# hhlgt/erasure-codes-prototype

Hardware: AMD Instinct MI355X
Metric: GiB/s encode + single-block decode (device-resident), RS(10,4) 1 MiB blocks, 1 & 8 GPU (higher is better)
Workload: dtype u8; 1 GPU; RS(10,4) encode + rotating 1-erasure decode (e = s mod 14); block_size=1048576, stripes_per_gpu=4096, global_stripes=4096, parallelism=stripes sharded over 1 GPU(s), no data-path collective

## Files before the change

erasure-codes-prototype_amd/csrc/gf_device.hpp:

```cpp
#pragma once
#include "gf_kernels.hpp"

namespace ecg {

#define ECG_CONST __attribute__((address_space(4)))
template <typename T>
__device__ __forceinline__ const ECG_CONST T* cst(const T* p) {
    return (const ECG_CONST T*)p;
}

template <int MODE>
__device__ __forceinline__ const uint8_t* src_ptr(const GfLaunch& a, int s, int prog, int j) {
    if constexpr (MODE == GF_MODE_INLINE || MODE == GF_MODE_INLINE_LAT) {
        return a.isrc[j];
    } else if constexpr (MODE == GF_MODE_PTRS) {
        return cst(a.src_ptrs)[(size_t)s * a.k + j];
    } else {
        const long long sa = a.stripe_of ? (long long)cst(a.stripe_of)[s] : (long long)s;
        return a.in_base + sa * a.in_sstride + (long long)cst(a.src_ids)[prog * a.k + j] * a.in_bstride;
    }
}

__device__ __forceinline__ uint32_t perm(uint32_t hi, uint32_t lo, uint32_t sel) {
    return __builtin_amdgcn_perm(hi, lo, sel);
}

__device__ __forceinline__ uint32_t xor3(uint32_t a, uint32_t b, uint32_t c) {
    return __builtin_amdgcn_bitop3_b32(a, b, c, 0x96);
}

typedef uint32_t u32x4 __attribute__((ext_vector_type(4)));

template <int NT>
__device__ __forceinline__ void load16(const uint8_t* p, uint32_t (&x)[4]) {
    u32x4 v;
    if constexpr (NT & 1) v = __builtin_nontemporal_load(reinterpret_cast<const u32x4*>(p));
    else v = *reinterpret_cast<const u32x4*>(p);
    x[0] = v.x; x[1] = v.y; x[2] = v.z; x[3] = v.w;
}

struct Split {
    uint32_t i0, i1, i2;
};

__device__ __forceinline__ Split split(uint32_t x) {
    return {x & 0x07070707u, (x >> 3) & 0x07070707u, (x >> 6) & 0x03030303u};
}

__device__ __forceinline__ uint32_t gmul(const ECG_CONST CoefTab& t, const Split& s) {
    return xor3(perm(t.t0hi, t.t0lo, s.i0), perm(t.t1hi, t.t1lo, s.i1), perm(t.t2, t.t2, s.i2));
}

template <int MT, int U>
__device__ __forceinline__ void fold_general(const uint32_t (&x)[U][4], const ECG_CONST CoefTab* t,
                                             uint32_t (&acc)[MT][4]) {
#pragma unroll
    for (int u = 0; u + 1 < U; u += 2) {
#pragma unroll
        for (int d = 0; d < 4; ++d) {
            const Split s0 = split(x[u][d]);
            const Split s1 = split(x[u + 1][d]);
#pragma unroll
            for (int p = 0; p < MT; ++p)
                acc[p][d] = xor3(acc[p][d], gmul(t[u * MT + p], s0), gmul(t[(u + 1) * MT + p], s1));
        }
    }
    if constexpr (U & 1) {
#pragma unroll
        for (int d = 0; d < 4; ++d) {
            const Split s0 = split(x[U - 1][d]);
#pragma unroll
            for (int p = 0; p < MT; ++p) acc[p][d] ^= gmul(t[(U - 1) * MT + p], s0);
        }
    }
}

template <int MT, int U>
__device__ __forceinline__ void fold_binary(const uint32_t (&x)[U][4], const ECG_CONST CoefTab* t,
                                            uint32_t (&acc)[MT][4]) {
#pragma unroll
    for (int u = 0; u < U; ++u)
#pragma unroll
        for (int p = 0; p < MT; ++p) {
            const uint32_t msk = t[u * MT + p].mask;
#pragma unroll
            for (int d = 0; d < 4; ++d) acc[p][d] = __builtin_amdgcn_bitop3_b32(acc[p][d], x[u][d], msk, 0x78);
        }
}

template <int MT, int U, bool BIN>
__device__ __forceinline__ void fold(const uint32_t (&x)[U][4], const ECG_CONST CoefTab* t, uint32_t (&acc)[MT][4]) {
    if constexpr (BIN) fold_binary<MT, U>(x, t, acc);
    else fold_general<MT, U>(x, t, acc);
}

constexpr int occupancy_for(int MT) {
#ifdef ECG_OCC_OVERRIDE
    return MT <= 4 ? ECG_OCC_OVERRIDE : 4;
#else
    return MT <= 2 ? 8 : MT <= 4 ? 6 : MT == 5 ? 3 : 4;
#endif
}

__device__ __forceinline__ void wg_coords(const GfLaunch& a, int& s, int& w) {
    long long b = blockIdx.x;
    if (a.grid_map == 1) {
        const long long G = (long long)gridDim.x;
        const long long per = G >> 3;
        b = (b & 7) * per + (b >> 3);
    } else if (a.grid_map == 2) {
        const long long i = b >> 3;
        const long long ls = i / a.wg_per_stripe;
        const long long G = a.map_group;
        s = (int)(((ls / G) * 8 + (b & 7)) * G + ls % G);
        w = (int)(i - ls * a.wg_per_stripe);
        return;
    }
    s = (int)(b / a.wg_per_stripe);
    w = (int)(b - (long long)s * a.wg_per_stripe);
}

template <int MODE>
__device__ __forceinline__ int launch_prog(const GfLaunch& a, int& s) {
    int r = 0;
    if constexpr (MODE == GF_MODE_STRIDED) {
        if (a.row_split) {
            r = s % a.row_split;
            s = s / a.row_split;
        }
    }
    const int p = a.prog_of_stripe ? cst(a.prog_of_stripe)[s] : 0;
    if constexpr (MODE == GF_MODE_STRIDED) return a.row_split ? p * a.row_split + r : p;
    return p;
}

#ifdef ECG_TUNE_LOAD_BATCH
constexpr int kLoadBatch = ECG_TUNE_LOAD_BATCH;
#else
constexpr int kLoadBatch = 4;
#endif
#ifdef ECG_TUNE_GEN_WIDE_LB
constexpr int kGenWideLB = ECG_TUNE_GEN_WIDE_LB;
#else
constexpr int kGenWideLB = 2;
#endif
#ifdef ECG_TUNE_GEN_LB
constexpr int kGenLB = ECG_TUNE_GEN_LB;
#else
constexpr int kGenLB = 4;
#endif

}
```

erasure-codes-prototype_amd/csrc/gf_kernels.hip:

```cpp
#include <atomic>

#include "gf_kernels.hpp"
#include "gf256.hpp"

#if defined(__HIP_DEVICE_COMPILE__) && !defined(__gfx950__)
#error "gf_kernels.hip is gfx950 (CDNA4) code"
#endif

#include "gf_done_flag.hpp"
#include "gf_device.hpp"

namespace ecg {

namespace {

template <int MODE>
__device__ __forceinline__ uint8_t* dst_ptr(const GfLaunch& a, int s, int prog, int p) {
    if constexpr (MODE == GF_MODE_INLINE || MODE == GF_MODE_INLINE_LAT) {
        return a.idst[p];
    } else if constexpr (MODE == GF_MODE_PTRS) {
        return cst(a.dst_ptrs)[(size_t)s * a.m + p];
    } else {
        const long long sa = a.stripe_of ? (long long)cst(a.stripe_of)[s] : (long long)s;
        return a.out_base + sa * a.out_sstride + (long long)cst(a.dst_ids)[prog * a.m + p] * a.out_bstride;
    }
}

template <int NT>
__device__ __forceinline__ void store16(uint8_t* p, const uint32_t (&x)[4]) {
    u32x4 v;
    v.x = x[0]; v.y = x[1]; v.z = x[2]; v.w = x[3];
    if constexpr (NT & 2) __builtin_nontemporal_store(v, reinterpret_cast<u32x4*>(p));
    else *reinterpret_cast<u32x4*>(p) = v;
}

template <int MT, int MODE, int NT, bool BIN>
__global__ void __launch_bounds__(kThreads, MODE == GF_MODE_INLINE_LAT ? 1 : occupancy_for(MT)) gf_vec_kernel(const GfLaunch a) {
    int s, w;
    wg_coords(a, s, w);
    const int rt = blockIdx.y;
    const int prog = launch_prog<MODE>(a, s);
    const int k = a.k;
    const int row0 = rt * MT;
    const int nrows = min(MT, a.m - row0);
    const ECG_CONST CoefTab* T = cst(a.tabs) + (size_t)(prog * a.rtiles + rt) * (size_t)k * MT;
    const long long ncols = a.B >> 4;
    const long long c0 = (long long)w * a.cols_per_wg;
    const long long c1 = min(c0 + (long long)a.cols_per_wg, ncols);

    uint8_t* dst[MT];
#pragma unroll
    for (int p = 0; p < MT; ++p) dst[p] = (p < nrows) ? dst_ptr<MODE>(a, s, prog, row0 + p) : nullptr;

    for (long long c = c0 + threadIdx.x; c < c1; c += kThreads) {
        const long long off = c << 4;
        uint32_t acc[MT][4];
#pragma unroll
        for (int p = 0; p < MT; ++p)
#pragma unroll
            for (int d = 0; d < 4; ++d) acc[p][d] = 0u;

        int j = 0;
        if constexpr (MODE == GF_MODE_INLINE_LAT) {
            if (k <= 8) {
                uint32_t x[8][4];
#pragma unroll
                for (int u = 0; u < 8; ++u) load16<NT>(src_ptr<MODE>(a, s, prog, u < k ? u : 0) + off, x[u]);
#pragma unroll
                for (int u = 0; u < 8; ++u)
                    if (u < k) fold<MT, 1, BIN>(reinterpret_cast<const uint32_t(&)[1][4]>(x[u]), T + (size_t)u * MT, acc);
                j = k;
            } else if (k <= 16) {
                uint32_t x[16][4];
#pragma unroll
                for (int u = 0; u < 16; ++u) load16<NT>(src_ptr<MODE>(a, s, prog, u < k ? u : 0) + off, x[u]);
#pragma unroll
                for (int u = 0; u < 16; ++u)
                    if (u < k) fold<MT, 1, BIN>(reinterpret_cast<const uint32_t(&)[1][4]>(x[u]), T + (size_t)u * MT, acc);
                j = k;
            }
        }
        constexpr int LB = BIN ? kLoadBatch : MT >= 5 ? kGenWideLB : kGenLB;
        for (; j + LB <= k; j += LB) {
            uint32_t x[LB][4];
#pragma unroll
            for (int u = 0; u < LB; ++u) load16<NT>(src_ptr<MODE>(a, s, prog, j + u) + off, x[u]);
            fold<MT, LB, BIN>(x, T + (size_t)j * MT, acc);
        }
        if constexpr (LB > 4) {
            if (j + 4 <= k) {
                uint32_t x[4][4];
#pragma unroll
                for (int u = 0; u < 4; ++u) load16<NT>(src_ptr<MODE>(a, s, prog, j + u) + off, x[u]);
                fold<MT, 4, BIN>(x, T + (size_t)j * MT, acc);
                j += 4;
            }
        }
        if (j + 2 <= k) {
            uint32_t x[2][4];
#pragma unroll
            for (int u = 0; u < 2; ++u) load16<NT>(src_ptr<MODE>(a, s, prog, j + u) + off, x[u]);
            fold<MT, 2, BIN>(x, T + (size_t)j * MT, acc);
            j += 2;
        }
        if (j < k) {
            uint32_t x[1][4];
            load16<NT>(src_ptr<MODE>(a, s, prog, j) + off, x[0]);
            fold<MT, 1, BIN>(x, T + (size_t)j * MT, acc);
        }
#pragma unroll
        for (int p = 0; p < MT; ++p)
            if (p < nrows) store16<NT>(dst[p] + off, acc[p]);
    }
    if constexpr (MODE == GF_MODE_INLINE_LAT) {
        if (a.done_flags) post_done_flag(a);
    }
}

template <int MT, int KB>
struct LatTabs {
    static constexpr int kPieces = KB * MT * 2;
    static constexpr int kPerLane = (kPieces + 63) / 64;
    CoefTab t[kLatThreads / 64][KB * MT];
};

template <int KB, int MT>
struct LatArgs {
    const CoefTab* tabs;
    unsigned* done_flags;
    long long B;
    int k, m;
    unsigned done_seq;
    const uint8_t* src[KB];
    uint8_t* dst[MT];
};

template <int MT, int KB>
__device__ __forceinline__ void lat_tabs_load(const LatArgs<KB, MT>& a, u32x4 (&tv)[LatTabs<MT, KB>::kPerLane]) {
    const u32x4* src = reinterpret_cast<const u32x4*>(a.tabs);
    const int last = a.k * MT * 2 - 1;
    const int lane = threadIdx.x & 63;
#pragma unroll
    for (int i = 0; i < LatTabs<MT, KB>::kPerLane; ++i) tv[i] = src[min(lane + 64 * i, last)];
}

template <int MT, int KB>
__device__ __forceinline__ const CoefTab* lat_tabs_store(LatTabs<MT, KB>& lds,
                                                         const u32x4 (&tv)[LatTabs<MT, KB>::kPerLane]) {
    const int wave = threadIdx.x >> 6, lane = threadIdx.x & 63;
    u32x4* dst = reinterpret_cast<u32x4*>(lds.t[wave]);
#pragma unroll
    for (int i = 0; i < LatTabs<MT, KB>::kPerLane; ++i)
        if (lane + 64 * i < LatTabs<MT, KB>::kPieces) dst[lane + 64 * i] = tv[i];
    return lds.t[wave];
}

template <int MT, bool BIN, int KB>
__device__ __forceinline__ void lat_fold_lds(const int k, const CoefTab* T, const uint32_t (&x)[KB],
                                             uint32_t (&acc)[MT]) {
    struct R {
        uint32_t t0lo, t0hi, t1lo, t1hi, t2;
    };
    auto rd = [&](int u, R (&r)[MT]) {
        const CoefTab* t = T + (size_t)(u < k ? u : 0) * MT;
#pragma unroll
        for (int p = 0; p < MT; ++p) {
            if constexpr (BIN) r[p].t0lo = t[p].mask;
            else r[p] = {t[p].t0lo, t[p].t0hi, t[p].t1lo, t[p].t1hi, t[p].t2};
        }
    };
#pragma unroll
    for (int p = 0; p < MT; ++p) acc[p] = 0u;
    R cur[MT], nxt[MT];
    rd(0, cur);
#pragma unroll
    for (int u = 0; u < KB; ++u) {
        if (u + 1 < KB) rd(u + 1, nxt);
        const uint32_t keep = u < k ? ~0u : 0u;
        if constexpr (BIN) {
#pragma unroll
            for (int p = 0; p < MT; ++p) acc[p] = __builtin_amdgcn_bitop3_b32(acc[p], x[u], cur[p].t0lo & keep, 0x78);
        } else {
            const Split sp = split(x[u]);
#pragma unroll
            for (int p = 0; p < MT; ++p) {
                const uint32_t g = xor3(perm(cur[p].t0hi, cur[p].t0lo, sp.i0), perm(cur[p].t1hi, cur[p].t1lo, sp.i1),
                                        perm(cur[p].t2, cur[p].t2, sp.i2));
                acc[p] = __builtin_amdgcn_bitop3_b32(acc[p], g, keep, 0x78);
            }
        }
#pragma unroll
        for (int p = 0; p < MT; ++p) asm volatile("" : "+v"(acc[p]) : : "memory");
        if (u + 1 < KB)
#pragma unroll
            for (int p = 0; p < MT; ++p) cur[p] = nxt[p];
    }
}

__device__ __forceinline__ void lat_store(uint32_t* p, uint32_t v) {
#ifdef ECG_TUNE_LAT_STORE_SC1
    asm volatile("global_store_dword %0, %1, off sc0 sc1" ::"v"(p), "v"(v) : "memory");
#else
    __builtin_nontemporal_store(v, p);
#endif
}

template <int MT, bool BIN, int KB, bool EAGER>
__global__ void __launch_bounds__(kLatThreads, 1) gf_lat_dword_kernel(const LatArgs<KB, MT> a) {
    __shared__ LatTabs<MT, KB> lds;
    const int k = a.k;
    const int nrows = a.m;
    const long long ndw = a.B >> 2;
    const long long c = (long long)blockIdx.x * kLatThreads + threadIdx.x;
    const uint8_t* src[KB];
#pragma unroll
    for (int u = 0; u < KB; ++u) src[u] = a.src[u];
    uint8_t* dst[MT];
#pragma unroll
    for (int p = 0; p < MT; ++p) dst[p] = a.dst[p];
    unsigned* const flags = a.done_flags;
    u32x4 tv[LatTabs<MT, KB>::kPerLane];
    lat_tabs_load<MT, KB>(a, tv);
    __builtin_amdgcn_sched_barrier(0);
    const bool live = c < ndw;
    const long long off = (live ? c : ndw - 1) << 2;
    uint32_t x[KB];
#pragma unroll
    for (int u = 0; u < KB; ++u) x[u] = __builtin_nontemporal_load(reinterpret_cast<const uint32_t*>(src[u] + off));
    if constexpr (EAGER) __builtin_amdgcn_sched_barrier(0);
    const CoefTab* T = lat_tabs_store<MT, KB>(lds, tv);
    uint32_t acc[MT];
    lat_fold_lds<MT, BIN, KB>(k, T, x, acc);
    if (live) {
#pragma unroll
        for (int p = 0; p < MT; ++p)
            if (p < nrows) lat_store(reinterpret_cast<uint32_t*>(dst[p] + off), acc[p]);
    }
    if (flags) post_done_flag(flags + blockIdx.x, a.done_seq);
}


__device__ __forceinline__ unsigned long long wk_ptr(const unsigned* d, int q) {
    return ((unsigned long long)d[worker_pos(q + 1)] << 32) | d[worker_pos(q)];
}

template <int MT, bool BIN, int KB>
__device__ __forceinline__ void worker_call(const unsigned* d, CoefTab* wt) {
    const int k = (int)d[worker_pos(WF_K)];
    const int m = (int)d[worker_pos(WF_M)];
    const long long ndw = (long long)d[worker_pos(WF_B)] >> 2;
    const u32x4* tg = reinterpret_cast<const u32x4*>((uintptr_t)wk_ptr(d, WF_TABS));
    const uint8_t* in[KB];
#pragma unroll
    for (int u = 0; u < KB; u++) in[u] = (const uint8_t*)(uintptr_t)wk_ptr(d, WF_IN + 2 * (u < k ? u : 0));
    uint8_t* out[MT];
#pragma unroll
    for (int p = 0; p < MT; p++) out[p] = (uint8_t*)(uintptr_t)wk_ptr(d, WF_OUT + 2 * (p < m ? p : 0));
    constexpr int kPieces = KB * MT * 2, kPerLane = (kPieces + 63) / 64;
    const int last = k * MT * 2 - 1, lane = threadIdx.x & 63;
    u32x4 tv[kPerLane];
#pragma unroll
    for (int i = 0; i < kPerLane; ++i) tv[i] = tg[min(lane + 64 * i, last)];
    __builtin_amdgcn_sched_barrier(0);
    const long long stride = (long long)gridDim.x * kLatThreads;
    long long c = (long long)blockIdx.x * kLatThreads + threadIdx.x;
    const bool live = c < ndw;
    uint32_t x[KB];
#pragma unroll
    for (int u = 0; u < KB; u++) x[u] = __builtin_nontemporal_load(reinterpret_cast<const uint32_t*>(in[u]) + (live ? c : 0));
#pragma unroll
    for (int i = 0; i < kPerLane; ++i)
        if (lane + 64 * i < kPieces) reinterpret_cast<u32x4*>(wt)[lane + 64 * i] = tv[i];
    uint32_t acc[MT];
    lat_fold_lds<MT, BIN, KB>(k, wt, x, acc);
    if (live) {
#pragma unroll
        for (int p = 0; p < MT; p++)
            if (p < m) __builtin_nontemporal_store(acc[p], reinterpret_cast<uint32_t*>(out[p]) + c);
    }
    for (c += stride; c < ndw; c += stride) {
#pragma unroll
        for (int u = 0; u < KB; u++) x[u] = __builtin_nontemporal_load(reinterpret_cast<const uint32_t*>(in[u]) + c);
        lat_fold_lds<MT, BIN, KB>(k, wt, x, acc);
#pragma unroll
        for (int p = 0; p < MT; p++)
            if (p < m) __builtin_nontemporal_store(acc[p], reinterpret_cast<uint32_t*>(out[p]) + c);
    }
}

template <int MT, bool BIN>
__device__ __forceinline__ void worker_call_k(const unsigned* d, CoefTab* wt) {
    const unsigned k = d[worker_pos(WF_K)];
    if (k <= 4) worker_call<MT, BIN, 4>(d, wt);
    else if (k <= 6) worker_call<MT, BIN, 6>(d, wt);
    else if (k <= 8) worker_call<MT, BIN, 8>(d, wt);
    else if (k <= 10) worker_call<MT, BIN, 10>(d, wt);
    else if (k <= 12) worker_call<MT, BIN, 12>(d, wt);
    else worker_call<MT, BIN, 16>(d, wt);
}

template <bool BIN>
__device__ __forceinline__ void worker_call_m(const unsigned* d, CoefTab* wt) {
    switch (d[worker_pos(WF_M)]) {
        case 1: worker_call_k<1, BIN>(d, wt); break;
        case 2: worker_call_k<2, BIN>(d, wt); break;
        case 3: worker_call_k<3, BIN>(d, wt); break;
        default: worker_call_k<4, BIN>(d, wt); break;
    }
}

__global__ void __launch_bounds__(kLatThreads, 1) gf_call_worker_kernel(const WorkerArgs a) {
    __shared__ unsigned d[64];
    __shared__ unsigned go;
    __shared__ CoefTab wtabs[kLatThreads / 64][kWorkerMaxSrc * kWorkerMaxRows];
    const int tid = threadIdx.x;
    const bool leader = blockIdx.x == 0;
    unsigned next = a.start_seq;
    const unsigned long long t0 = wall_clock64();
    unsigned long long last = t0;
    const unsigned long long my_idle = leader ? a.idle_ticks : 2 * a.idle_ticks;
    const unsigned long long my_life = leader ? a.life_ticks : 2 * a.life_ticks;
    for (unsigned polls = 0; polls < a.max_polls; polls++) {
        const unsigned slot = next % (unsigned)kWorkerSlots;
        if (leader) {
            if (tid < 64) {
                const unsigned v = __hip_atomic_load(&a.ring[slot].w[tid], __ATOMIC_RELAXED, __HIP_MEMORY_SCOPE_SYSTEM);
                const unsigned stop = __hip_atomic_load(a.stop, __ATOMIC_RELAXED, __HIP_MEMORY_SCOPE_SYSTEM);
                d[tid] = v;
                if (tid == 0) go = stop ? 2u : 0u;
            }
            __syncthreads();
            if (tid == 0 && go == 0) {
                const unsigned long long t = wall_clock64();
                if (t - t0 > my_life) go = 2;
                else if (d[0] == next && d[16] == next && d[32] == next && d[48] == next) go = 1;
                else if (t - last > my_idle) go = 2;
            }
            __syncthreads();
            if (go == 1 && gridDim.x > 1 && tid < 64) {
                __hip_atomic_store(&a.mbox[slot].w[tid], d[tid], __ATOMIC_RELAXED, __HIP_MEMORY_SCOPE_AGENT);
                if (tid == 0) __hip_atomic_store(&a.mbseq[slot], next, __ATOMIC_RELEASE, __HIP_MEMORY_SCOPE_AGENT);
            }
        } else {
            if (tid == 0) {
                const unsigned sq = __hip_atomic_load(&a.mbseq[slot], __ATOMIC_ACQUIRE, __HIP_MEMORY_SCOPE_AGENT);
                const unsigned ex = __hip_atomic_load(&a.mbseq[kWorkerSlots], __ATOMIC_RELAXED, __HIP_MEMORY_SCOPE_AGENT);
                const unsigned long long t = wall_clock64();
                go = sq == next ? 1u : (ex == a.gen || t - last > my_idle || t - t0 > my_life) ? 2u : 0u;
            }
            __syncthreads();
            if (go == 1 && tid < 64)
                d[tid] = __hip_atomic_load(&a.mbox[slot].w[tid], __ATOMIC_RELAXED, __HIP_MEMORY_SCOPE_AGENT);
            __syncthreads();
        }
        const unsigned g = go;
        if (g == 2) break;
        if (g == 0) {
            __syncthreads();
            continue;
        }
        __builtin_amdgcn_fence(__ATOMIC_ACQUIRE, "");
        CoefTab* const wt = wtabs[tid >> 6];
        if (d[worker_pos(WF_BINARY)]) worker_call_m<true>(d, wt);
        else worker_call_m<false>(d, wt);
        post_done_flag(a.flags + (size_t)slot * kWorkerMaxWG + blockIdx.x, next);
        next++;
        last = wall_clock64();
        __syncthreads();
    }
    if (tid == 0) {
        if (leader) __hip_atomic_store(&a.mbseq[kWorkerSlots], a.gen, __ATOMIC_RELAXED, __HIP_MEMORY_SCOPE_AGENT);
        __hip_atomic_store(a.exit_info + blockIdx.x, a.gen, __ATOMIC_RELAXED, __HIP_MEMORY_SCOPE_SYSTEM);
    }
}

template <int MT, int MODE, bool BIN>
__global__ void __launch_bounds__(kThreads) gf_byte_kernel(const GfLaunch a) {
    int s, w;
    wg_coords(a, s, w);
    const int rt = blockIdx.y;
    const int prog = launch_prog<MODE>(a, s);
    const int k = a.k;
    const int row0 = rt * MT;
    const int nrows = min(MT, a.m - row0);
    const ECG_CONST CoefTab* T = cst(a.tabs) + (size_t)(prog * a.rtiles + rt) * (size_t)k * MT;
    const long long b0 = a.off0 + (long long)w * a.cols_per_wg;
    const long long b1 = min(b0 + (long long)a.cols_per_wg, a.B);
    for (long long o = b0 + threadIdx.x; o < b1; o += kThreads) {
        uint32_t acc[MT];
#pragma unroll
        for (int p = 0; p < MT; ++p) acc[p] = 0u;
        for (int j = 0; j < k; ++j) {
            const uint32_t x = src_ptr<MODE>(a, s, prog, j)[o];
            const ECG_CONST CoefTab* t = T + (size_t)j * MT;
            if constexpr (BIN) {
#pragma unroll
                for (int p = 0; p < MT; ++p) acc[p] ^= x & t[p].mask;
            } else {
                const Split sp = split(x);
#pragma unroll
                for (int p = 0; p < MT; ++p) acc[p] ^= gmul(t[p], sp);
            }
        }
#pragma unroll
        for (int p = 0; p < MT; ++p)
            if (p < nrows) dst_ptr<MODE>(a, s, prog, row0 + p)[o] = (uint8_t)(acc[p] & 0xffu);
    }
}

__global__ void __launch_bounds__(kThreads) fill_splitmix_kernel(uint8_t* dst, long long nbytes,
                                                                 unsigned long long seed,
                                                                 unsigned long long word_offset) {
    const long long nwords = nbytes >> 3;
    const long long stride = (long long)gridDim.x * kThreads;
    for (long long w = (long long)blockIdx.x * kThreads + threadIdx.x; w < ((nbytes + 7) >> 3); w += stride) {
        unsigned long long z = seed + (word_offset + (unsigned long long)w) * 0x9E3779B97F4A7C15ull;
        z = (z ^ (z >> 30)) * 0xBF58476D1CE4E5B9ull;
        z = (z ^ (z >> 27)) * 0x94D049BB133111EBull;
        z ^= z >> 31;
        if (w < nwords) {
            reinterpret_cast<unsigned long long*>(dst)[w] = z;
        } else {
            for (long long b = w * 8; b < nbytes; ++b) dst[b] = (uint8_t)(z >> (8 * (b - w * 8)));
        }
    }
}


std::atomic<long long> g_opt[ECG_OPT_COUNT] = {};
std::atomic<int> g_opt_init{0};

void init_options() {
    if (g_opt_init.load(std::memory_order_acquire)) return;
    auto env = [](const char* n, long long d) {
        const char* e = getenv(n);
        return e ? atoll(e) : d;
    };
    g_opt[ECG_OPT_NT].store(env("ECG_NT", 3));
    g_opt[ECG_OPT_COLS_PER_WG].store(env("ECG_COLS_PER_WG", 0));
    g_opt[ECG_OPT_GRID_MAP].store(env("ECG_GRID_MAP", 3));
    g_opt[ECG_OPT_ZEROCOPY_BYTES].store(env("ECG_ZEROCOPY_BYTES", 8 << 20));
    g_opt[ECG_OPT_PROGRAM_CACHE].store(env("ECG_PROGRAM_CACHE", 4096));
    g_opt[ECG_OPT_MAP_GROUP].store(env("ECG_MAP_GROUP", 1));
    g_opt[ECG_OPT_LAT_DWORD_BYTES].store(env("ECG_LAT_DWORD_BYTES", 1 << 20));
    g_opt[ECG_OPT_CALL_WORKER].store(env("ECG_CALL_WORKER", 0));
    g_opt[ECG_OPT_ROW_SPLIT].store(env("ECG_ROW_SPLIT", 16));
    g_opt[ECG_OPT_GRAVEYARD].store(env("ECG_GRAVEYARD", 16384));
    g_opt[ECG_OPT_MT1_LDS_PAD].store(env("ECG_MT1_LDS_PAD", -1));
    g_opt_init.store(1, std::memory_order_release);
}

using Launcher = hipError_t (*)(const GfLaunch&, dim3, hipStream_t);

template <typename T>
struct NoDeduce {
    using type = T;
};

template <typename... P>
hipError_t launch_kernel_lds(void (*kernel)(P...), dim3 grid, dim3 block, unsigned lds, hipStream_t st,
                             typename NoDeduce<P>::type... args) {
    void* argv[] = {(void*)&args...};
    return hipLaunchKernel((const void*)kernel, grid, block, argv, lds, st);
}

template <typename... P>
hipError_t launch_kernel(void (*kernel)(P...), dim3 grid, dim3 block, hipStream_t st,
                         typename NoDeduce<P>::type... args) {
    return launch_kernel_lds(kernel, grid, block, 0, st, args...);
}

template <typename F>
hipError_t launch_with(F kernel, const GfLaunch& a, dim3 grid, hipStream_t st) {
    return launch_kernel(kernel, grid, dim3(kThreads), st, a);
}

unsigned mt1_lds_pad(int k, bool ptrs) {
    const long long opt = g_opt[ECG_OPT_MT1_LDS_PAD].load(std::memory_order_relaxed);
    if (opt >= 0) return (unsigned)opt;
    if (k <= 1) return 0;
    if (k <= 3) return 12288;
    if (k == 4) return 16384;
    if (k == 5) return 0;
    if (k == 6) return ptrs ? 22528 : 20480;
    if (k == 7 || k == 9 || k == 10) return 22528;
    return 24576;
}

unsigned mt2_lds_pad(int k) {
#ifdef ECG_TUNE_PAD_MT2
    const long long opt = g_opt[ECG_OPT_MT1_LDS_PAD].load(std::memory_order_relaxed);
    if (opt >= 0) return (unsigned)opt;
#endif
    return k <= 7 ? 0u : k <= 11 ? 20480u : 24576u;
}

template <int MT, int MODE, int NT, bool BIN>
hipError_t gen_launch(const GfLaunch& a, dim3 g, hipStream_t st) {
#ifdef ECG_TUNE_PAD_MT_LO
    if constexpr (MT >= ECG_TUNE_PAD_MT_LO && MT <= ECG_TUNE_PAD_MT_HI) {
        const long long opt = g_opt[ECG_OPT_MT1_LDS_PAD].load(std::memory_order_relaxed);
        return launch_kernel_lds(gf_vec_kernel<MT, MODE, NT, BIN>, g, dim3(kThreads), opt > 0 ? (unsigned)opt : 0u, st, a);
    }
#endif
    constexpr bool kWideBinCap = BIN && (MT == 8 || MT == 9);
    const unsigned lds = MT == 1 ? mt1_lds_pad(a.k, MODE == GF_MODE_PTRS)
                         : MT == 2 ? mt2_lds_pad(a.k)
                         : (kWideBinCap && a.k >= 12) ? 20480u : 0u;
    return launch_kernel_lds(gf_vec_kernel<MT, MODE, NT, BIN>, g, dim3(kThreads), lds, st, a);
}

template <int MODE, int NT, bool BIN>
Launcher gen_pick(int MT) {
    switch (MT) {
        case 1: return gen_launch<1, MODE, NT, BIN>;
        case 2: return gen_launch<2, MODE, NT, BIN>;
        case 3: return gen_launch<3, MODE, NT, BIN>;
        case 4: return gen_launch<4, MODE, NT, BIN>;
        case 5: return gen_launch<5, MODE, NT, BIN>;
        case 6: return gen_launch<6, MODE, NT, BIN>;
        case 7: return gen_launch<7, MODE, NT, BIN>;
        case 8: return gen_launch<8, MODE, NT, BIN>;
        default: break;
    }
    if constexpr (BIN && NT == 3) {
        switch (MT) {
            case 9: return gen_launch<9, MODE, NT, BIN>;
            case 10: return gen_launch<10, MODE, NT, BIN>;
            case 11: return gen_launch<11, MODE, NT, BIN>;
            case 12: return gen_launch<12, MODE, NT, BIN>;
            case 13: return gen_launch<13, MODE, NT, BIN>;
            case 14: return gen_launch<14, MODE, NT, BIN>;
            case 15: return gen_launch<15, MODE, NT, BIN>;
            case 16: return gen_launch<16, MODE, NT, BIN>;
            default: break;
        }
    }
    return nullptr;
}

template <int MODE, int NT>
Launcher pick_vec_nt(const GfLaunch& a) {
    return a.binary ? gen_pick<MODE, NT, true>(a.MT) : gen_pick<MODE, NT, false>(a.MT);
}

template <int MODE>
Launcher pick_vec(const GfLaunch& a, int nt) {
    switch (nt & 3) {
        case 0: return pick_vec_nt<MODE, 0>(a);
        case 1: return pick_vec_nt<MODE, 1>(a);
        case 2: return pick_vec_nt<MODE, 2>(a);
        default: return pick_vec_nt<MODE, 3>(a);
    }
}

template <int MT, bool BIN, int KB>
hipError_t lat_dword_launch(const GfLaunch& a, dim3 g, hipStream_t st) {
    LatArgs<KB, MT> l;
    l.tabs = a.tabs;
    l.done_flags = a.done_flags;
    l.B = a.B;
    l.k = a.k;
    l.m = a.m;
    l.done_seq = a.done_seq;
    for (int u = 0; u < KB; ++u) l.src[u] = a.isrc[u < a.k ? u : 0];
    for (int p = 0; p < MT; ++p) l.dst[p] = a.idst[p < a.m ? p : 0];
    if (a.B <= kLatEagerBytes) return launch_kernel(gf_lat_dword_kernel<MT, BIN, KB, true>, g, dim3(kLatThreads), st, l);
    return launch_kernel(gf_lat_dword_kernel<MT, BIN, KB, false>, g, dim3(kLatThreads), st, l);
}

template <int MT, bool BIN>
Launcher pick_lat_k(int k) {
    if (k <= 4) return lat_dword_launch<MT, BIN, 4>;
    if (k <= 6) return lat_dword_launch<MT, BIN, 6>;
    if (k <= 8) return lat_dword_launch<MT, BIN, 8>;
    if (k <= 10) return lat_dword_launch<MT, BIN, 10>;
    if (k <= 12) return lat_dword_launch<MT, BIN, 12>;
    if (k <= 16) return lat_dword_launch<MT, BIN, 16>;
    return nullptr;
}

template <bool BIN>
Launcher pick_lat_dword_bin(int MT, int k) {
    switch (MT) {
        case 1: return pick_lat_k<1, BIN>(k);
        case 2: return pick_lat_k<2, BIN>(k);
        case 3: return pick_lat_k<3, BIN>(k);
        case 4: return pick_lat_k<4, BIN>(k);
        case 5: return pick_lat_k<5, BIN>(k);
        case 6: return pick_lat_k<6, BIN>(k);
        case 7: return pick_lat_k<7, BIN>(k);
        case 8: return pick_lat_k<8, BIN>(k);
        default: return nullptr;
    }
}

template <int MT, int MODE, bool BIN>
hipError_t byte_launch(const GfLaunch& a, dim3 g, hipStream_t st) {
    return launch_with(gf_byte_kernel<MT, MODE, BIN>, a, g, st);
}

template <int MODE, bool BIN>
Launcher pick_byte_bin(int MT) {
    switch (MT) {
        case 1: return byte_launch<1, MODE, BIN>;
        case 2: return byte_launch<2, MODE, BIN>;
        case 3: return byte_launch<3, MODE, BIN>;
        case 4: return byte_launch<4, MODE, BIN>;
        case 5: return byte_launch<5, MODE, BIN>;
        case 6: return byte_launch<6, MODE, BIN>;
        case 7: return byte_launch<7, MODE, BIN>;
        case 8: return byte_launch<8, MODE, BIN>;
        default: break;
    }
    if constexpr (BIN) {
        switch (MT) {
            case 9: return byte_launch<9, MODE, BIN>;
            case 10: return byte_launch<10, MODE, BIN>;
            case 11: return byte_launch<11, MODE, BIN>;
            case 12: return byte_launch<12, MODE, BIN>;
            case 13: return byte_launch<13, MODE, BIN>;
            case 14: return byte_launch<14, MODE, BIN>;
            case 15: return byte_launch<15, MODE, BIN>;
            case 16: return byte_launch<16, MODE, BIN>;
            default: break;
        }
    }
    return nullptr;
}

template <int MODE>
Launcher pick_byte(const GfLaunch& a) {
    return a.binary ? pick_byte_bin<MODE, true>(a.MT) : pick_byte_bin<MODE, false>(a.MT);
}

}

long long get_option(int opt) {
    init_options();
    if (opt < 0 || opt >= ECG_OPT_COUNT) return -1;
    return g_opt[opt].load();
}

int set_option(int opt, long long value) {
    init_options();
    if (opt < 0 || opt >= ECG_OPT_COUNT) return -1;
    if (opt == ECG_OPT_NT && (value < 0 || value > 3)) return -1;
    if (opt == ECG_OPT_COLS_PER_WG && (value < 0 || (value % kThreads) != 0)) return -1;
    if (opt == ECG_OPT_GRID_MAP && (value < 0 || value > 3)) return -1;
    if (opt == ECG_OPT_ZEROCOPY_BYTES && value < 0) return -1;
    if (opt == ECG_OPT_PROGRAM_CACHE && value < 2) return -1;
    if (opt == ECG_OPT_MAP_GROUP && (value < 1 || value > (1 << 20))) return -1;
    if (opt == ECG_OPT_LAT_DWORD_BYTES && value < 0) return -1;
    if (opt == ECG_OPT_CALL_WORKER && (value < 0 || value > 1000000)) return -1;
    if (opt == ECG_OPT_ROW_SPLIT && value < 0) return -1;
    if (opt == ECG_OPT_GRAVEYARD && value < 1) return -1;
    if (opt == ECG_OPT_MT1_LDS_PAD && (value < -1 || value > 65536)) return -1;
    g_opt[opt].store(value);
    return 0;
}

static bool outputs_in_stripe(const GfLaunch& a, int mode) {
    if (mode == GF_MODE_PTRS) return a.grid_map != 2;
    if (mode != GF_MODE_STRIDED) return true;
    const uint8_t* o = a.out_base;
    return a.out_sstride == a.in_sstride && o >= a.in_base && o < a.in_base + a.in_sstride;
}

std::atomic<long long> g_launched{0}, g_moved{0};

void launch_traffic(long long* launches, long long* bytes) {
    if (launches) *launches = g_launched.load(std::memory_order_relaxed);
    if (bytes) *bytes = g_moved.load(std::memory_order_relaxed);
}

static_assert(GF_MODE_INLINE == 0 && GF_MODE_PTRS == 1 && GF_MODE_STRIDED == 2 && GF_MODE_INLINE_LAT == 3,
              "ECG_HIST_* slots are laid out by these mode numbers");
static_assert(kMaxMTBin == 16 && kMaxMT <= kMaxMTBin, "ECG_HIST_* slots hold 16 tile widths");
std::atomic<long long> g_hist[ECG_HIST_SLOTS] = {};

static void hist_vec(int mode, int binary, int nt, int MT) {
    g_hist[ECG_HIST_VEC + (((mode * 2 + (binary ? 1 : 0)) * 4 + (nt & 3)) * 16 + (MT - 1))].fetch_add(
        1, std::memory_order_relaxed);
}

static void hist_byte(int mode, int binary, int MT) {
    g_hist[ECG_HIST_BYTE + ((mode * 2 + (binary ? 1 : 0)) * 16 + (MT - 1))].fetch_add(1, std::memory_order_relaxed);
}

static void hist_lat(int binary, int MT, int k, long long B) {
    const int kb = k <= 4 ? 0 : k <= 6 ? 1 : k <= 8 ? 2 : k <= 10 ? 3 : k <= 12 ? 4 : 5;
    g_hist[ECG_HIST_LAT + ((((binary ? 1 : 0) * 8 + (MT - 1)) * 6 + kb) * 2 + (B <= kLatEagerBytes ? 1 : 0))].fetch_add(
        1, std::memory_order_relaxed);
}

int launch_histogram(long long* counts, int cap) {
    for (int i = 0; counts && i < cap && i < ECG_HIST_SLOTS; i++) counts[i] = g_hist[i].load(std::memory_order_relaxed);
    return ECG_HIST_SLOTS;
}

hipError_t launch_gf(const GfLaunch& base, int mode, bool vec_ok, hipStream_t st, int* n_wg) {
    if (n_wg) *n_wg = 0;
    if (base.k < 1 || base.m < 1 || base.S < 1 || base.B < 0 || base.MT < 1 ||
        base.MT > (base.binary ? kMaxMTBin : kMaxMT))
        return hipErrorInvalidValue;
    if ((mode == GF_MODE_INLINE || mode == GF_MODE_INLINE_LAT) &&
        (base.S != 1 || base.k > kInlineSrc || base.m > kInlineDst))
        return hipErrorInvalidValue;
    if (base.B == 0) return hipSuccess;
    init_options();
    GfLaunch a = base;
    const long long vec_bytes = vec_ok ? (a.B & ~15LL) : 0;
    g_launched.fetch_add((vec_bytes > 0) + (vec_bytes < a.B), std::memory_order_relaxed);
    g_moved.fetch_add((long long)a.S * a.B * ((long long)a.rtiles * a.k + a.m), std::memory_order_relaxed);
    if (mode == GF_MODE_INLINE_LAT && vec_bytes == a.B && a.B <= g_opt[ECG_OPT_LAT_DWORD_BYTES].load() &&
        a.k <= kLatMaxSrc && a.rtiles == 1 && a.MT <= kMaxMT) {
        const long long gx = ((a.B >> 2) + kLatThreads - 1) / kLatThreads;
        Launcher l = a.binary ? pick_lat_dword_bin<true>(a.MT, a.k) : pick_lat_dword_bin<false>(a.MT, a.k);
        if (!l) return hipErrorInvalidValue;
        hist_lat(a.binary, a.MT, a.k, a.B);
        const hipError_t e = l(a, dim3((unsigned)gx), st);
        if (e != hipSuccess) return e;
        if (n_wg) *n_wg = (int)gx;
        return hipSuccess;
    }
    if (vec_bytes > 0) {
        const long long ncols = vec_bytes >> 4;
        long long cpw = g_opt[ECG_OPT_COLS_PER_WG].load();
        if (cpw <= 0) cpw = kThreads;
        if (ncols < cpw) cpw = ((ncols + kThreads - 1) / kThreads) * kThreads;
        a.cols_per_wg = (int)cpw;
        a.wg_per_stripe = (int)((ncols + cpw - 1) / cpw);
        a.off0 = 0;
        const long long gx = (long long)a.S * a.wg_per_stripe;
        if (gx > 0x7fffffffLL) return hipErrorInvalidConfiguration;
        long long gm = g_opt[ECG_OPT_GRID_MAP].load();
        if (gm == 3) gm = outputs_in_stripe(a, mode) ? 1 : 2;
        long long G = g_opt[ECG_OPT_MAP_GROUP].load();
        while (G > 1 && a.S % (8 * G) != 0) G >>= 1;
        if (gm == 2 && a.S % (8 * G) != 0) gm = 1;
        a.grid_map = (gm == 1 && gx % 8 == 0) ? 1 : (gm == 2) ? 2 : 0;
        a.map_group = (int)G;
        const int nt = a.MT > kMaxMT ? 3 : (int)g_opt[ECG_OPT_NT].load();
        Launcher l = nullptr;
        switch (mode) {
            case GF_MODE_INLINE: l = pick_vec<GF_MODE_INLINE>(a, nt); break;
            case GF_MODE_INLINE_LAT: l = pick_vec<GF_MODE_INLINE_LAT>(a, nt); break;
            case GF_MODE_PTRS: l = pick_vec<GF_MODE_PTRS>(a, nt); break;
            case GF_MODE_STRIDED: l = pick_vec<GF_MODE_STRIDED>(a, nt); break;
            default: return hipErrorInvalidValue;
        }
        if (!l) return hipErrorInvalidValue;
        if (a.done_flags && (mode != GF_MODE_INLINE_LAT || vec_bytes < a.B)) return hipErrorInvalidValue;
        hist_vec(mode, a.binary, nt, a.MT);
        const hipError_t e = l(a, dim3((unsigned)gx, (unsigned)a.rtiles), st);
        if (e != hipSuccess) return e;
        if (n_wg) *n_wg = (int)(gx * a.rtiles);
    }
    if (a.done_flags && vec_bytes < a.B) return hipErrorInvalidValue;
    if (vec_bytes < a.B) {
        const long long nbytes = a.B - vec_bytes;
        long long bpw = 16LL * kThreads;
        if (nbytes < bpw) bpw = ((nbytes + kThreads - 1) / kThreads) * kThreads;
        a.cols_per_wg = (int)bpw;
        a.wg_per_stripe = (int)((nbytes + bpw - 1) / bpw);
        a.off0 = vec_bytes;
        a.grid_map = 0;
        const long long gx = (long long)a.S * a.wg_per_stripe;
        if (gx > 0x7fffffffLL) return hipErrorInvalidConfiguration;
        Launcher l = nullptr;
        switch (mode) {
            case GF_MODE_INLINE:
            case GF_MODE_INLINE_LAT: l = pick_byte<GF_MODE_INLINE>(a); break;
            case GF_MODE_PTRS: l = pick_byte<GF_MODE_PTRS>(a); break;
            case GF_MODE_STRIDED: l = pick_byte<GF_MODE_STRIDED>(a); break;
            default: return hipErrorInvalidValue;
        }
        if (!l) return hipErrorInvalidValue;
        hist_byte(mode == GF_MODE_INLINE_LAT ? (int)GF_MODE_INLINE : mode, a.binary, a.MT);
        const hipError_t e = l(a, dim3((unsigned)gx, (unsigned)a.rtiles), st);
        if (e != hipSuccess) return e;
    }
    return hipSuccess;
}

hipError_t launch_call_worker(const WorkerArgs& a, int workgroups, hipStream_t st) {
    if (workgroups < 1 || workgroups > kWorkerMaxWG) return hipErrorInvalidValue;
    return launch_kernel(gf_call_worker_kernel, dim3((unsigned)workgroups), dim3(kLatThreads), st, a);
}

hipError_t launch_fill_splitmix(void* dst, long long nbytes, unsigned long long seed,
                                unsigned long long word_offset, hipStream_t st) {
    if (nbytes <= 0) return hipSuccess;
    const long long nwords = (nbytes + 7) >> 3;
    long long blocks = (nwords + kThreads - 1) / kThreads;
    if (blocks > 8192) blocks = 8192;
    return launch_kernel(fill_splitmix_kernel, dim3((unsigned)blocks), dim3(kThreads), st, (uint8_t*)dst, nbytes,
                         seed, word_offset);
}

void make_coef_tab(int c, CoefTab* t) {
    c &= 0xff;
    uint8_t e0[8], e1[8], e2[4];
    for (int e = 0; e < 8; ++e) {
        e0[e] = (uint8_t)gf::mul(c, e);
        e1[e] = (uint8_t)gf::mul(c, e << 3);
    }
    for (int e = 0; e < 4; ++e) e2[e] = (uint8_t)gf::mul(c, e << 6);
    auto pack = [](const uint8_t* b) {
        return (uint32_t)b[0] | ((uint32_t)b[1] << 8) | ((uint32_t)b[2] << 16) | ((uint32_t)b[3] << 24);
    };
    t->t0lo = pack(e0);
    t->t0hi = pack(e0 + 4);
    t->t1lo = pack(e1);
    t->t1hi = pack(e1 + 4);
    t->t2 = pack(e2);
    t->mask = (c == 1) ? 0xffffffffu : 0u;
    t->pad0 = 0u;
    t->pad1 = 0u;
}

}
```

erasure-codes-prototype_amd/csrc/gf_kernels.hpp:

```cpp
#pragma once
#include <hip/hip_runtime.h>
#include <stdint.h>

#include "../../include/ecg.h"

namespace ecg {

struct alignas(32) CoefTab {
    uint32_t t0lo, t0hi;
    uint32_t t1lo, t1hi;
    uint32_t t2;
    uint32_t mask;
    uint32_t pad0, pad1;
};

enum GfMode : int {
    GF_MODE_INLINE = 0,
    GF_MODE_PTRS = 1,
    GF_MODE_STRIDED = 2,
    GF_MODE_INLINE_LAT = 3,
};

constexpr int kInlineSrc = 128;
constexpr int kInlineDst = 32;
constexpr int kMaxMT = 8;
constexpr int kMaxMTBin = 16;
#ifndef ECG_TPB
#define ECG_TPB 128
#endif
constexpr int kLatThreads = 256;
constexpr int kLatMaxSrc = 16;
constexpr long long kLatEagerBytes = 16 << 10;
constexpr int kThreads = ECG_TPB;

struct GfLaunch {
    const CoefTab* tabs;
    const int* src_ids;
    const int* dst_ids;
    const int* prog_of_stripe;
    const int* stripe_of;
    int row_split;
    const uint8_t* in_base;
    uint8_t* out_base;
    long long in_sstride, in_bstride, out_sstride, out_bstride;
    const uint8_t* const* src_ptrs;
    uint8_t* const* dst_ptrs;
    const uint8_t* isrc[kInlineSrc];
    uint8_t* idst[kInlineDst];
    long long B;
    long long off0;
    int k, m, S;
    int MT, rtiles;
    int binary;
    int grid_map;
    int map_group;
    int wg_per_stripe;
    int cols_per_wg;
    unsigned* done_flags;
    unsigned done_seq;
};

constexpr int kWorkerSlots = 4;
constexpr int kWorkerMaxWG = 16;
constexpr int kWorkerMaxSrc = 16;
constexpr int kWorkerMaxRows = 4;
struct alignas(256) WorkerDesc {
    unsigned w[64];
};
enum WorkerField : int {
    WF_K = 0, WF_M = 1, WF_B = 2, WF_BINARY = 3, WF_TABS = 4,
    WF_IN = 8,
    WF_OUT = WF_IN + 2 * kWorkerMaxSrc,
    WF_END = WF_OUT + 2 * kWorkerMaxRows
};
static_assert(WF_END <= 60, "worker payload fits 60 dwords");
__host__ __device__ constexpr int worker_pos(int q) { return q + 1 + q / 15; }

struct WorkerArgs {
    const WorkerDesc* ring;
    unsigned* flags;
    const unsigned* stop;
    WorkerDesc* mbox;
    unsigned* mbseq;
    unsigned* exit_info;
    unsigned start_seq, gen, max_polls;
    unsigned long long idle_ticks, life_ticks;
};
hipError_t launch_call_worker(const WorkerArgs& a, int workgroups, hipStream_t stream);

long long get_option(int opt);
int set_option(int opt, long long value);

hipError_t launch_gf(const GfLaunch& base, int mode, bool vec_ok, hipStream_t stream, int* n_wg = nullptr);
void launch_traffic(long long* launches, long long* bytes);
int launch_histogram(long long* counts, int cap);

hipError_t launch_fill_splitmix(void* dst, long long nbytes, unsigned long long seed,
                                unsigned long long word_offset, hipStream_t stream);

void make_coef_tab(int c, CoefTab* out);

}
```

Before: 4745 GiB/s.

## Precompute per-workgroup addressing with reciprocal division and vectorized pointer loads

Replaces 64-bit divides in workgroup coordinate mapping with host-precomputed 32-bit reciprocal multiplies. Source and destination pointers or ids are now fetched as vector loads from constant memory per batch, and stores use explicit global address-space pointers. The aim is to cut scalar address-setup overhead in the GF vector kernel. It adds new GfLaunch fields and a correction step in the fast divide. The div_rcp value for d<=1 relies on that correction step to stay exact.

```diff
diff --git a/erasure-codes-prototype_amd/csrc/gf_device.hpp b/erasure-codes-prototype_amd/csrc/gf_device.hpp
--- a/erasure-codes-prototype_amd/csrc/gf_device.hpp
+++ b/erasure-codes-prototype_amd/csrc/gf_device.hpp
@@ -134,6 +134,102 @@
     return p;
 }
 
+
+__device__ __forceinline__ uint32_t fast_div(uint32_t n, uint32_t d, uint32_t rcp) {
+    const uint32_t q = __umulhi(n, rcp);
+    return q + (n - q * d >= d ? 1u : 0u);
+}
+
+struct WgAddr {
+    int w, prog;
+    const uint8_t* in;
+    uint8_t* out;
+    const ECG_CONST uint32_t* ids;
+    const ECG_CONST uint32_t* oids;
+};
+
+template <int MODE>
+__device__ __forceinline__ WgAddr wg_addr(const GfLaunch& a) {
+    WgAddr g;
+    uint32_t b = blockIdx.x, s;
+    const uint32_t wps = (uint32_t)a.wg_per_stripe;
+    if (a.grid_map == 2) {
+        const uint32_t i = b >> 3, G = (uint32_t)a.map_group;
+        const uint32_t ls = fast_div(i, wps, a.rcp_wg_per_stripe);
+        const uint32_t lg = fast_div(ls, G, a.rcp_map_group);
+        s = (lg * 8u + (b & 7u)) * G + (ls - lg * G);
+        g.w = (int)(i - ls * wps);
+    } else {
+        if (a.grid_map == 1) b = (b & 7u) * (gridDim.x >> 3) + (b >> 3);
+        s = fast_div(b, wps, a.rcp_wg_per_stripe);
+        g.w = (int)(b - s * wps);
+    }
+    uint32_t r = 0;
+    if constexpr (MODE == GF_MODE_STRIDED) {
+        if (a.row_split) {
+            const uint32_t q = fast_div(s, (uint32_t)a.row_split, a.rcp_row_split);
+            r = s - q * (uint32_t)a.row_split;
+            s = q;
+        }
+    }
+    int p = a.prog_of_stripe ? cst(a.prog_of_stripe)[s] : 0;
+    if constexpr (MODE == GF_MODE_STRIDED) {
+        if (a.row_split) p = p * a.row_split + (int)r;
+    }
+    g.prog = p;
+    if constexpr (MODE == GF_MODE_STRIDED) {
+        const long long sa = a.stripe_of ? (long long)cst(a.stripe_of)[s] : (long long)s;
+        g.in = a.in_base + sa * a.in_sstride;
+        g.out = a.out_base + sa * a.out_sstride;
+        g.ids = (const ECG_CONST uint32_t*)cst(a.src_ids) + (size_t)p * a.k;
+        g.oids = (const ECG_CONST uint32_t*)cst(a.dst_ids) + (size_t)p * a.m;
+    } else if constexpr (MODE == GF_MODE_PTRS) {
+        g.in = nullptr;
+        g.out = nullptr;
+        g.ids = (const ECG_CONST uint32_t*)(cst(a.src_ptrs) + (size_t)s * a.k);
+        g.oids = (const ECG_CONST uint32_t*)(cst(a.dst_ptrs) + (size_t)s * a.m);
+    } else {
+        g.in = nullptr;
+        g.out = nullptr;
+        g.ids = (const ECG_CONST uint32_t*)cst(a.isrc);
+        g.oids = (const ECG_CONST uint32_t*)cst(a.idst);
+    }
+    return g;
+}
+
+template <int N>
+struct IdVec {
+    typedef uint32_t type __attribute__((ext_vector_type(N), aligned(4)));
+};
+template <>
+struct IdVec<1> {
+    typedef uint32_t type;
+};
+
+template <int N>
+__device__ __forceinline__ uint32_t id_elem(const typename IdVec<N>::type& v, int i) {
+    if constexpr (N == 1) return v;
+    else return v[i];
+}
+
+template <int MODE, int U, typename P>
+__device__ __forceinline__ void batch_ptrs(const ECG_CONST uint32_t* row, P* base, long long bstride, int j,
+                                           P* (&ptr)[U]) {
+    constexpr int N = MODE == GF_MODE_STRIDED ? U : 2 * U;
+    typedef typename IdVec<N>::type V;
+    const V v = *(const ECG_CONST V*)(row + (MODE == GF_MODE_STRIDED ? j : 2 * j));
+#pragma unroll
+    for (int u = 0; u < U; ++u) {
+        if constexpr (MODE == GF_MODE_STRIDED) {
+            ptr[u] = base + (long long)(int)id_elem<N>(v, u) * bstride;
+        } else {
+            typedef P __attribute__((address_space(1))) * GlobalPtr;
+            ptr[u] = (P*)(GlobalPtr)(uintptr_t)(((unsigned long long)id_elem<N>(v, 2 * u + 1) << 32) |
+                                                id_elem<N>(v, 2 * u));
+        }
+    }
+}
+
 #ifdef ECG_TUNE_LOAD_BATCH
 constexpr int kLoadBatch = ECG_TUNE_LOAD_BATCH;
 #else
diff --git a/erasure-codes-prototype_amd/csrc/gf_kernels.hip b/erasure-codes-prototype_amd/csrc/gf_kernels.hip
--- a/erasure-codes-prototype_amd/csrc/gf_kernels.hip
+++ b/erasure-codes-prototype_amd/csrc/gf_kernels.hip
@@ -28,29 +28,48 @@
 
 template <int NT>
 __device__ __forceinline__ void store16(uint8_t* p, const uint32_t (&x)[4]) {
+    typedef u32x4 __attribute__((address_space(1))) * GlobalVec;
     u32x4 v;
     v.x = x[0]; v.y = x[1]; v.z = x[2]; v.w = x[3];
-    if constexpr (NT & 2) __builtin_nontemporal_store(v, reinterpret_cast<u32x4*>(p));
-    else *reinterpret_cast<u32x4*>(p) = v;
+    if constexpr (NT & 2) __builtin_nontemporal_store(v, (GlobalVec)p);
+    else *(GlobalVec)p = v;
+}
+
+template <int MT, int U, int MODE, int NT, bool BIN>
+__device__ __forceinline__ void load_fold(const WgAddr& g, long long bstride, int j, long long off,
+                                          const ECG_CONST CoefTab* T, uint32_t (&acc)[MT][4]) {
+    const uint8_t* p[U];
+    batch_ptrs<MODE, U>(g.ids, g.in, bstride, j, p);
+    uint32_t x[U][4];
+#pragma unroll
+    for (int u = 0; u < U; ++u) load16<NT>(p[u] + off, x[u]);
+    fold<MT, U, BIN>(x, T + (size_t)j * MT, acc);
 }
 
 template <int MT, int MODE, int NT, bool BIN>
 __global__ void __launch_bounds__(kThreads, MODE == GF_MODE_INLINE_LAT ? 1 : occupancy_for(MT)) gf_vec_kernel(const GfLaunch a) {
-    int s, w;
-    wg_coords(a, s, w);
+    const WgAddr g = wg_addr<MODE>(a);
     const int rt = blockIdx.y;
-    const int prog = launch_prog<MODE>(a, s);
     const int k = a.k;
     const int row0 = rt * MT;
     const int nrows = min(MT, a.m - row0);
-    const ECG_CONST CoefTab* T = cst(a.tabs) + (size_t)(prog * a.rtiles + rt) * (size_t)k * MT;
+    const ECG_CONST CoefTab* T = cst(a.tabs) + (size_t)(g.prog * a.rtiles + rt) * (size_t)k * MT;
     const long long ncols = a.B >> 4;
-    const long long c0 = (long long)w * a.cols_per_wg;
+    const long long c0 = (long long)g.w * a.cols_per_wg;
     const long long c1 = min(c0 + (long long)a.cols_per_wg, ncols);
+    const long long ibs = a.in_bstride;
 
     uint8_t* dst[MT];
-#pragma unroll
-    for (int p = 0; p < MT; ++p) dst[p] = (p < nrows) ? dst_ptr<MODE>(a, s, prog, row0 + p) : nullptr;
+    if ((MT & (MT - 1)) == 0 && nrows == MT) {
+        if constexpr ((MT & (MT - 1)) == 0) batch_ptrs<MODE, MT>(g.oids, g.out, a.out_bstride, row0, dst);
+    } else {
+#pragma unroll
+        for (int p = 0; p < MT; ++p) {
+            uint8_t* one[1];
+            batch_ptrs<MODE, 1>(g.oids, g.out, a.out_bstride, row0 + min(p, nrows - 1), one);
+            dst[p] = one[0];
+        }
+    }
 
     for (long long c = c0 + threadIdx.x; c < c1; c += kThreads) {
         const long long off = c << 4;
@@ -65,7 +84,7 @@
             if (k <= 8) {
                 uint32_t x[8][4];
 #pragma unroll
-                for (int u = 0; u < 8; ++u) load16<NT>(src_ptr<MODE>(a, s, prog, u < k ? u : 0) + off, x[u]);
+                for (int u = 0; u < 8; ++u) load16<NT>(src_ptr<MODE>(a, 0, 0, u < k ? u : 0) + off, x[u]);
 #pragma unroll
                 for (int u = 0; u < 8; ++u)
                     if (u < k) fold<MT, 1, BIN>(reinterpret_cast<const uint32_t(&)[1][4]>(x[u]), T + (size_t)u * MT, acc);
@@ -73,7 +92,7 @@
             } else if (k <= 16) {
                 uint32_t x[16][4];
 #pragma unroll
-                for (int u = 0; u < 16; ++u) load16<NT>(src_ptr<MODE>(a, s, prog, u < k ? u : 0) + off, x[u]);
+                for (int u = 0; u < 16; ++u) load16<NT>(src_ptr<MODE>(a, 0, 0, u < k ? u : 0) + off, x[u]);
 #pragma unroll
                 for (int u = 0; u < 16; ++u)
                     if (u < k) fold<MT, 1, BIN>(reinterpret_cast<const uint32_t(&)[1][4]>(x[u]), T + (size_t)u * MT, acc);
@@ -81,33 +100,20 @@
             }
         }
         constexpr int LB = BIN ? kLoadBatch : MT >= 5 ? kGenWideLB : kGenLB;
-        for (; j + LB <= k; j += LB) {
-            uint32_t x[LB][4];
-#pragma unroll
-            for (int u = 0; u < LB; ++u) load16<NT>(src_ptr<MODE>(a, s, prog, j + u) + off, x[u]);
-            fold<MT, LB, BIN>(x, T + (size_t)j * MT, acc);
-        }
+        for (; j + LB <= k; j += LB) load_fold<MT, LB, MODE, NT, BIN>(g, ibs, j, off, T, acc);
         if constexpr (LB > 4) {
             if (j + 4 <= k) {
-                uint32_t x[4][4];
-#pragma unroll
-                for (int u = 0; u < 4; ++u) load16<NT>(src_ptr<MODE>(a, s, prog, j + u) + off, x[u]);
-                fold<MT, 4, BIN>(x, T + (size_t)j * MT, acc);
+                load_fold<MT, 4, MODE, NT, BIN>(g, ibs, j, off, T, acc);
                 j += 4;
             }
         }
-        if (j + 2 <= k) {
-            uint32_t x[2][4];
-#pragma unroll
-            for (int u = 0; u < 2; ++u) load16<NT>(src_ptr<MODE>(a, s, prog, j + u) + off, x[u]);
-            fold<MT, 2, BIN>(x, T + (size_t)j * MT, acc);
-            j += 2;
-        }
-        if (j < k) {
-            uint32_t x[1][4];
-            load16<NT>(src_ptr<MODE>(a, s, prog, j) + off, x[0]);
-            fold<MT, 1, BIN>(x, T + (size_t)j * MT, acc);
-        }
+        if constexpr (LB > 2) {
+            if (j + 2 <= k) {
+                load_fold<MT, 2, MODE, NT, BIN>(g, ibs, j, off, T, acc);
+                j += 2;
+            }
+        }
+        if (j < k) load_fold<MT, 1, MODE, NT, BIN>(g, ibs, j, off, T, acc);
 #pragma unroll
         for (int p = 0; p < MT; ++p)
             if (p < nrows) store16<NT>(dst[p] + off, acc[p]);
@@ -741,6 +747,9 @@
         if (gm == 2 && a.S % (8 * G) != 0) gm = 1;
         a.grid_map = (gm == 1 && gx % 8 == 0) ? 1 : (gm == 2) ? 2 : 0;
         a.map_group = (int)G;
+        a.rcp_wg_per_stripe = div_rcp((uint32_t)a.wg_per_stripe);
+        a.rcp_map_group = div_rcp((uint32_t)a.map_group);
+        a.rcp_row_split = div_rcp((uint32_t)a.row_split);
         const int nt = a.MT > kMaxMT ? 3 : (int)g_opt[ECG_OPT_NT].load();
         Launcher l = nullptr;
         switch (mode) {
diff --git a/erasure-codes-prototype_amd/csrc/gf_kernels.hpp b/erasure-codes-prototype_amd/csrc/gf_kernels.hpp
--- a/erasure-codes-prototype_amd/csrc/gf_kernels.hpp
+++ b/erasure-codes-prototype_amd/csrc/gf_kernels.hpp
@@ -56,9 +56,12 @@
     int map_group;
     int wg_per_stripe;
     int cols_per_wg;
+    uint32_t rcp_wg_per_stripe, rcp_map_group, rcp_row_split;
     unsigned* done_flags;
     unsigned done_seq;
 };
+
+constexpr uint32_t div_rcp(uint32_t d) { return d <= 1 ? 0xffffffffu : (uint32_t)((1ull << 32) / d); }
 
 constexpr int kWorkerSlots = 4;
 constexpr int kWorkerMaxWG = 16;
```

Result: no change. 4703 GiB/s (-0.9%).
